# george-gca/sr-pytorch-lightning

Measured on AMD Instinct MI355X. Metric: SR training throughput, LR patches/s (48x48 LR x4, fwd+bwd+Adam), higher is better.
Workload: dtype bf16; 1 GPU; edsr_baseline x4, 48x48 LR patches, batch 256/GPU, train step (L1 + Adam); global_batch=256, parallelism=dp1, hip_graph=full

## Files before the change

### sr-pytorch-lightning_amd/csrc/conv_wgrad.hip

```cpp
#include <stdlib.h>
#include "srk_common.h"

namespace {

template <int DT, int KS> struct WgCfg {
  typedef DTraits<DT> Tr;
  static constexpr int CH = Tr::CH;
  static constexpr int ESZ = 16 / CH;
  static constexpr int CBLK = 128 / ESZ;
  static constexpr int RB = CBLK / 32;
  static constexpr int PAIRS = RB * RB;
  static constexpr int KGROUPS = 4 / PAIRS;
  static constexpr int NT = 256;
  static constexpr int NTAPS = KS * KS;
  static constexpr int PAD = KS / 2;
  static constexpr int TIN = 16 + KS - 1;
  static constexpr int PITCH = (TIN + 1) & ~1;
  static constexpr int XS_BYTES = TIN * PITCH * 128;
  static constexpr int DYS_BYTES = 256 * 128;
  static constexpr int LDS_BYTES = XS_BYTES + DYS_BYTES;
  static constexpr int XPIECES = TIN * TIN * 8;
  static constexpr int DYPIECES = 256 * 8;
};

// ... 52 lines not shown
    int pt = tile;
    const int tX = pt % tilesX;
    pt /= tilesX;
    const int tY = pt % tilesY;
    const int n = pt / tilesY;
    const int y0 = tY * 16, x0 = tX * 16;

    __syncthreads();
#pragma unroll 1
    for (int base = tid; base < C::XPIECES; base += 4 * C::NT) {
      i32x4 v[4];
#pragma unroll
      for (int u = 0; u < 4; ++u) {
        const int i = base + u * C::NT;
        v[u] = i32x4{0, 0, 0, 0};
        if (i < C::XPIECES) {
          const int s = i & 7, p = i >> 3;
          const int iy = p / C::TIN, ix = p - iy * C::TIN;
          const int c = cib * 8 + (s ^ swz(ix));
          const int gy = y0 + iy - C::PAD, gx = x0 + ix - C::PAD;
          if (c < nch_x && gy >= 0 && gy < H && gx >= 0 && gx < W)
            v[u] = gload16(xg + chunk_off(n, gy, gx, H, W, rx, Csx, c * CH, a.x_pitch, a.x_coff));
        }
      }
#pragma unroll
      for (int u = 0; u < 4; ++u) {
        const int i = base + u * C::NT;
        if (i < C::XPIECES) {
          const int s = i & 7, p = i >> 3;
          const int iy = p / C::TIN, ix = p - iy * C::TIN;
          lds_write16(Xs + ((iy * C::PITCH + ix) << 7) + (s << 4), v[u]);
        }
      }
    }
#pragma unroll 1
    for (int base = tid; base < C::DYPIECES; base += 4 * C::NT) {
      i32x4 v[4];
#pragma unroll
      for (int u = 0; u < 4; ++u) {
        const int i = base + u * C::NT;
        const int s = i & 7, p = i >> 3;
        const int iy = p >> 4, ix = p & 15;
        const int c = cob * 8 + (s ^ swz(ix));
        const int gy = y0 + iy, gx = x0 + ix;
        v[u] = i32x4{0, 0, 0, 0};
        if (c < nch_d && gy < H && gx < W)
          v[u] = gload16(dg + chunk_off(n, gy, gx, H, W, rd, Csd, c * CH, a.dy_pitch, a.dy_coff));
      }
#pragma unroll
      for (int u = 0; u < 4; ++u) lds_write16(Ds + ((base + u * C::NT) << 4), v[u]);
    }
    __syncthreads();

    if (a.dbp && cib == 0) {
#pragma unroll 4
      for (int p = b_part; p < 256; p += BPARTS) {
        const char* ad = Ds + (p << 7) + ((((b_c / CH)) ^ swz(p & 15)) << 4) + (b_c % CH) * C::ESZ;
        bsum += Tr::to_f32(*reinterpret_cast<const elem*>(ad));
      }
    }

    if constexpr (Tr::IS16) {
      i32x4 xf[KS][KS];
#pragma unroll
      for (int rr = 0; rr < KS - 1; ++rr)
#pragma unroll
        for (int kw = 0; kw < KS; ++kw)
          xf[rr % KS][kw] = tr_read2(Xs + xoff[kw][0] + rr * (C::PITCH * 128), Xs + xoff[kw][1] + rr * (C::PITCH * 128));
#pragma unroll
      for (int y = 0; y < 16; ++y) {
        const int nr = y + KS - 1;
#pragma unroll
        for (int kw = 0; kw < KS; ++kw)
          xf[nr % KS][kw] = tr_read2(Xs + xoff[kw][0] + nr * (C::PITCH * 128), Xs + xoff[kw][1] + nr * (C::PITCH * 128));
        const i32x4 bf = tr_read2(Ds + doff[0] + y * (16 * 128), Ds + doff[1] + y * (16 * 128));
#pragma unroll
        for (int t = 0; t < C::NTAPS; ++t) {
          const int kh = t / KS, kw = t - kh * KS;
          acc[t] = Tr::mma(xf[(y + kh) % KS][kw], bf, acc[t]);
        }
      }
    } else {
      const int i = lane & 31, hk = lane >> 5;
#pragma unroll 1
      for (int y = kgroup; y < 16; y += C::KGROUPS) {
#pragma unroll 2
        for (int m = 0; m < 8; ++m) {
          const int col = 2 * m + hk;
          const float b = lds_f32(Ds, 16, y, col, i);
#pragma unroll
          for (int t = 0; t < C::NTAPS; ++t) {
            const int kh = t / KS, kw = t - kh * KS;
            const float av = lds_f32(Xs, C::PITCH, y + kh, col + kw, i);
            acc[t] = __builtin_amdgcn_mfma_f32_32x32x2f32(av, b, acc[t], 0, 0, 0);
          }
        }
      }
    }
  }

  const int co = cob * C::CBLK + cbk * 32 + (lane & 31);
  const int hq = lane >> 5;
  if (co < a.Cout) {
#pragma unroll
    for (int t = 0; t < C::NTAPS; ++t) {
#pragma unroll
      for (int e = 0; e < 16; ++e) {
        const int ci = cib * C::CBLK + rb * 32 + (e & 3) + 8 * (e >> 2) + 4 * hq;
        if (ci < a.Cin) atomicAdd(a.dwp + ((size_t)t * a.Cin + ci) * a.Cout + co, acc[t][e]);
      }
    }
  }
  if (a.dbp && cib == 0) {
    const int c = cob * C::CBLK + b_c;
    if (c < a.Cout) atomicAdd(a.dbp + c, bsum);
  }
}


typedef __attribute__((address_space(3))) void lds_void_t;

template <int DT>
SRK_DEV void wgrad_ws_body16(const srk_wgrad_args& a, const int slot, const int cib, const int cob, const int tilesX, const int tilesY,
                           const unsigned x_bytes, const unsigned dy_bytes, const int tq, const int trem, char* const smem) {
  typedef WgCfg<DT, 3> C;
  typedef typename C::Tr Tr;
  typedef typename Tr::elem elem;
  constexpr int CH = C::CH, KS = 3, GT = 256, ESZ = C::ESZ;
  constexpr int NPK = (C::XPIECES + GT - 1) / GT;
  constexpr int NDK = C::DYPIECES / GT;
  constexpr int BUF_BYTES = C::XS_BYTES + C::DYS_BYTES;

  const int tid = threadIdx.x, lane = tid & 63;
  const int wave = __builtin_amdgcn_readfirstlane(tid >> 6);
  const int rb = wave >> 1, cbk = wave & 1;
  const int H = a.H, W = a.W;
  const int nch_x = a.Cin / CH, nch_d = a.Cout / CH;

  const int t0 = slot * tq + min(slot, trem);
  const int nt = tq + (slot < trem ? 1 : 0);

  const i32x4 xrs = make_rsrc4(a.x, x_bytes), drs = make_rsrc4(a.dy, dy_bytes);
  const unsigned lds0 = lds_addr_of(smem);
  int pconst[NPK], pyx[NPK];
#pragma unroll
  for (int k = 0; k < NPK; ++k) {
    const int i = tid + k * GT;
    const int sl = i & 7, p = i >> 3;
    const int iy = p / C::TIN, ix = p - iy * C::TIN;
    const int c = cib * 8 + (sl ^ swz(ix));
    pconst[k] = (((iy - 1) * W + (ix - 1)) * a.x_pitch + a.x_coff + c * CH) * ESZ;
    pyx[k] = (i < C::XPIECES && c < nch_x) ? (((iy - 1) & 0xffff) | ((ix - 1) << 16)) : (int)0x7fff7fff;
  }
  const int rd = a.dy_ps > 1 ? a.dy_ps : 1;
  const int d_ix = (tid >> 3) & 15, d_iy0 = tid >> 7;
  const int d_c = cob * 8 + ((tid & 7) ^ swz(d_ix));
  const bool d_cok = d_c < nch_d;
  int dconst, dkstride;
  {
    const int Csd = a.Cout / (rd * rd);
    const int k0 = d_c * CH;
    const int ij = k0 / Csd, c0 = k0 - ij * Csd;
    const int si = ij / rd, sj = ij - si * rd;
    dconst = (((d_iy0 * rd + si) * (W * rd) + d_ix * rd + sj) * a.dy_pitch + a.dy_coff + c0) * ESZ;
    dkstride = 2 * rd * (W * rd) * a.dy_pitch * ESZ;
  }
  struct TileAddr { int y0, x0, xbase, dbase; bool colok; unsigned Xb; };
  auto tile_addr = [&](int pt, char* Xb) {
    TileAddr t;
    const int tX = pt % tilesX;
    const int q = pt / tilesX;
    const int tY = q % tilesY, n = q / tilesY;
    t.y0 = tY * 16; t.x0 = tX * 16;
    t.xbase = (((n * H + t.y0) * W + t.x0) * a.x_pitch) * ESZ;
    t.dbase = (((n * H * rd + t.y0 * rd) * (W * rd) + t.x0 * rd) * a.dy_pitch) * ESZ;
    t.colok = d_cok && (t.x0 + d_ix < W);
    t.Xb = lds0 + (unsigned)(Xb - smem);
    return t;
  };
  auto dma_x_piece = [&](const TileAddr& t, int k) {
    const int gy = t.y0 + (int)(short)(pyx[k] & 0xffff), gx = t.x0 + (pyx[k] >> 16);
    const bool ok = (unsigned)gy < (unsigned)H && (unsigned)gx < (unsigned)W;
    const unsigned voff = ok ? (unsigned)(t.xbase + pconst[k]) : 0x80000000u;
    if (k < NPK - 1 || tid + k * GT < C::XPIECES)
      dma16_hidden(xrs, voff, __builtin_amdgcn_readfirstlane(t.Xb + ((k * GT + wave * 64) << 4)));
  };
  auto dma_d_piece = [&](const TileAddr& t, int k) {
    const bool ok = t.colok && (t.y0 + d_iy0 + 2 * k < H);
    const unsigned voff = ok ? (unsigned)(t.dbase + dconst + k * dkstride) : 0x80000000u;
    dma16_hidden(drs, voff, __builtin_amdgcn_readfirstlane(t.Xb + C::XS_BYTES + ((k * GT + wave * 64) << 4)));
  };
  auto dma_tile = [&](int pt, char* Xb) {
    const TileAddr t = tile_addr(pt, Xb);
#pragma unroll
    for (int k = 0; k < NPK; ++k) dma_x_piece(t, k);
#pragma unroll
    for (int k = 0; k < NDK; ++k) dma_d_piece(t, k);
  };

  f32x16 acc[9];
#pragma unroll
  for (int t = 0; t < 9; ++t)
#pragma unroll
    for (int e = 0; e < 16; ++e) acc[t][e] = 0.f;
  float bsum8[8] = {0.f, 0.f, 0.f, 0.f, 0.f, 0.f, 0.f, 0.f};
  const bool do_bias = a.dbp != nullptr && cib == 0;
  int xoff[KS][2], doff[2];
#pragma unroll
  for (int kw = 0; kw < KS; ++kw) {
    xoff[kw][0] = tr_lane_off(kw, 0, rb, lane);
    xoff[kw][1] = tr_lane_off(kw, 1, rb, lane);
  }
  doff[0] = tr_lane_off(0, 0, cbk, lane);
  doff[1] = tr_lane_off(0, 1, cbk, lane);

  dma_tile(t0, smem);
#pragma unroll 1
  for (int it = 0; it < nt; ++it) {
    char* const Xs = smem + (it & 1) * BUF_BYTES;
    char* const Ds = Xs + C::XS_BYTES;
    asm volatile("s_waitcnt vmcnt(0)" ::: "memory");
    __builtin_amdgcn_s_barrier();
    const bool more = it + 1 < nt;
    const TileAddr nxt = tile_addr(more ? t0 + it + 1 : t0 + it, smem + ((it + 1) & 1) * BUF_BYTES);

    if (do_bias) {
#pragma unroll
      for (int k = 0; k < 8; ++k) {
        const i32x4 raw = lds_read16(Ds + ((tid + 256 * k) << 4));
        const uint32_t w4[4] = {(uint32_t)raw.x, (uint32_t)raw.y, (uint32_t)raw.z, (uint32_t)raw.w};
#pragma unroll
        for (int i = 0; i < 4; ++i) {
          bsum8[2 * i] += Tr::to_f32((uint16_t)(w4[i] & 0xffff));
          bsum8[2 * i + 1] += Tr::to_f32((uint16_t)(w4[i] >> 16));
        }
      }
    }
    i32x4 xf[4][KS];
#pragma unroll
    for (int rr = 0; rr < 3; ++rr)
#pragma unroll
      for (int kw = 0; kw < KS; ++kw)
        xf[rr][kw] = tr_read2(Xs + xoff[kw][0] + rr * (C::PITCH * 128), Xs + xoff[kw][1] + rr * (C::PITCH * 128));
    i32x4 bf = tr_read2(Ds + doff[0], Ds + doff[1]);
#pragma unroll
    for (int y = 0; y < 16; ++y) {
      i32x4 bfn = bf;
      if (y + 1 < 16) {
        const int nr = y + 3;
#pragma unroll
        for (int kw = 0; kw < KS; ++kw)
          xf[nr & 3][kw] = tr_read2(Xs + xoff[kw][0] + nr * (C::PITCH * 128), Xs + xoff[kw][1] + nr * (C::PITCH * 128));
        bfn = tr_read2(Ds + doff[0] + (y + 1) * (16 * 128), Ds + doff[1] + (y + 1) * (16 * 128));
      }
#pragma unroll
      for (int t = 0; t < 9; ++t) {
        const int kh = t / KS, kw = t - kh * KS;
        acc[t] = Tr::mma(xf[(y + kh) & 3][kw], bf, acc[t]);
        if (t == 1 && 2 * y < NPK && more) dma_x_piece(nxt, 2 * y);
        if (t == 4 && 2 * y + 1 < NPK && more) dma_x_piece(nxt, 2 * y + 1);
        if (t == 7 && y < NDK && more) dma_d_piece(nxt, y);
      }
      bf = bfn;
      __builtin_amdgcn_sched_barrier(0);
    }
  }

  {
    const int co = cob * 64 + cbk * 32 + (lane & 31);
    const int hq = lane >> 5;
    const size_t slab_elems = (size_t)9 * a.Cin * a.Cout;
    const __amdgpu_buffer_rsrc_t srs =
        __builtin_amdgcn_make_buffer_rsrc(a.dwp + (size_t)slot * slab_elems, 0, (unsigned)(slab_elems * 4), 0x00020000);
    const int ci0 = cib * 64 + rb * 32 + 4 * hq;
#pragma unroll
    for (int t = 0; t < 9; ++t) {
#pragma unroll
      for (int e = 0; e < 16; ++e) {
        const int ci = ci0 + (e & 3) + 8 * (e >> 2);
        const unsigned voff = (ci < a.Cin && co < a.Cout) ? (unsigned)(((t * a.Cin + ci) * a.Cout + co) * 4) : 0x80000000u;
        __builtin_amdgcn_raw_buffer_store_b32(__float_as_uint(acc[t][e]), srs, voff, 0, 0);
      }
    }
  }
  if (do_bias) {
    float* const bred = reinterpret_cast<float*>(smem);
    __syncthreads();
#pragma unroll
    for (int e = 0; e < 8; ++e) bred[tid * 8 + e] = bsum8[e];
    __syncthreads();
    if (tid < 64) {
      const int ch = tid >> 3, e = tid & 7;
      float t = 0.f;
      for (int p0 = 0; p0 < 32; ++p0) t += bred[((p0 << 3) + (ch ^ swz(p0 & 15))) * 8 + e];
      const int c = cob * 64 + tid;
      if (c < a.Cout) a.dbp[(size_t)slot * a.Cout + c] = t;
    }
  }
}


constexpr int WS_TH = 8;

template <int DT>
SRK_DEV void wgrad_ws_body8(const srk_wgrad_args& a, const int slot, const int cib, const int cob, const int tilesX, const int tilesY,
                           const unsigned x_bytes, const unsigned dy_bytes, const int tq, const int trem, char* const smem) {
  typedef WgCfg<DT, 3> C;
  typedef typename C::Tr Tr;
  typedef typename Tr::elem elem;
  constexpr int CH = C::CH, KS = 3, GT = 256, ESZ = C::ESZ;
  constexpr int TH = WS_TH, NBUF = 4, AHEAD = NBUF - 1;
  constexpr int XPIECES = (TH + 2) * C::TIN * 8;
  constexpr int NPK = (XPIECES + GT - 1) / GT;
  constexpr int NDK = TH * 16 * 8 / GT;
  constexpr int PPT = NPK + NDK;
  constexpr int XS_PAD = NPK * GT * 16, DYS = TH * 16 * 128;
  constexpr int BUF_BYTES = XS_PAD + DYS;
  static_assert(NBUF * BUF_BYTES <= 160 * 1024, "the ring must fit the LDS");

  const int tid = threadIdx.x, lane = tid & 63;
  const int wave = __builtin_amdgcn_readfirstlane(tid >> 6);
  const int rb = wave >> 1, cbk = wave & 1;
  const int H = a.H, W = a.W;
  const int nch_x = a.Cin / CH, nch_d = a.Cout / CH;

  const int t0 = slot * tq + min(slot, trem);
  const int nt = tq + (slot < trem ? 1 : 0);

  const i32x4 xrs = make_rsrc4(a.x, x_bytes), drs = make_rsrc4(a.dy, dy_bytes);
  const unsigned lds0 = lds_addr_of(smem);
  int pconst[NPK], pyx[NPK];
#pragma unroll
  for (int k = 0; k < NPK; ++k) {
    const int i = tid + k * GT;
    const int sl = i & 7, p = i >> 3;
    const int iy = p / C::TIN, ix = p - iy * C::TIN;
    const int c = cib * 8 + (sl ^ swz(ix));
    pconst[k] = (((iy - 1) * W + (ix - 1)) * a.x_pitch + a.x_coff + c * CH) * ESZ;
    pyx[k] = (i < XPIECES && c < nch_x) ? (((iy - 1) & 0xffff) | ((ix - 1) << 16)) : (int)0x7fff7fff;
  }
  const int rd = a.dy_ps > 1 ? a.dy_ps : 1;
  const int d_ix = (tid >> 3) & 15, d_iy0 = tid >> 7;
  const int d_c = cob * 8 + ((tid & 7) ^ swz(d_ix));
  const bool d_cok = d_c < nch_d;
  int dconst, dkstride;
  {
    const int Csd = a.Cout / (rd * rd);
    const int k0 = d_c * CH;
    const int ij = k0 / Csd, c0 = k0 - ij * Csd;
    const int si = ij / rd, sj = ij - si * rd;
    dconst = (((d_iy0 * rd + si) * (W * rd) + d_ix * rd + sj) * a.dy_pitch + a.dy_coff + c0) * ESZ;
    dkstride = 2 * rd * (W * rd) * a.dy_pitch * ESZ;
  }
  struct TileAddr { int y0, x0, xbase, dbase; bool colok, live; unsigned Xb; };
  auto tile_addr = [&](int it_, char* Xb) {
    TileAddr t;
    t.live = it_ < nt;
    const int pt = t0 + (t.live ? it_ : 0);
    const int tX = pt % tilesX;
    const int q = pt / tilesX;
    const int tY = q % tilesY, n = q / tilesY;
    t.y0 = tY * TH; t.x0 = tX * 16;
    t.xbase = (((n * H + t.y0) * W + t.x0) * a.x_pitch) * ESZ;
    t.dbase = (((n * H * rd + t.y0 * rd) * (W * rd) + t.x0 * rd) * a.dy_pitch) * ESZ;
    t.colok = t.live && d_cok && (t.x0 + d_ix < W);
    t.Xb = lds0 + (unsigned)(Xb - smem);
    return t;
  };
  auto dma_x_piece = [&](const TileAddr& t, int k) {
    const int gy = t.y0 + (int)(short)(pyx[k] & 0xffff), gx = t.x0 + (pyx[k] >> 16);
    const bool ok = t.live && (unsigned)gy < (unsigned)H && (unsigned)gx < (unsigned)W;
    const unsigned voff = ok ? (unsigned)(t.xbase + pconst[k]) : 0x80000000u;
    dma16_hidden(xrs, voff, __builtin_amdgcn_readfirstlane(t.Xb + ((k * GT + wave * 64) << 4)));
  };
  auto dma_d_piece = [&](const TileAddr& t, int k) {
    const bool ok = t.colok && (t.y0 + d_iy0 + 2 * k < H);
    const unsigned voff = ok ? (unsigned)(t.dbase + dconst + k * dkstride) : 0x80000000u;
    dma16_hidden(drs, voff, __builtin_amdgcn_readfirstlane(t.Xb + XS_PAD + ((k * GT + wave * 64) << 4)));
  };
  auto dma_tile = [&](int it_, char* Xb) {
    const TileAddr t = tile_addr(it_, Xb);
#pragma unroll
    for (int k = 0; k < NPK; ++k) dma_x_piece(t, k);
#pragma unroll
    for (int k = 0; k < NDK; ++k) dma_d_piece(t, k);
  };

  f32x16 acc[9];
#pragma unroll
  for (int t = 0; t < 9; ++t)
#pragma unroll
    for (int e = 0; e < 16; ++e) acc[t][e] = 0.f;
  float bsum8[8] = {0.f, 0.f, 0.f, 0.f, 0.f, 0.f, 0.f, 0.f};
  const bool do_bias = a.dbp != nullptr && cib == 0;
  int xoff[KS][2], doff[2];
#pragma unroll
  for (int kw = 0; kw < KS; ++kw) {
    xoff[kw][0] = tr_lane_off(kw, 0, rb, lane);
    xoff[kw][1] = tr_lane_off(kw, 1, rb, lane);
  }
  doff[0] = tr_lane_off(0, 0, cbk, lane);
  doff[1] = tr_lane_off(0, 1, cbk, lane);

#pragma unroll
  for (int k = 0; k < AHEAD; ++k) dma_tile(k, smem + k * BUF_BYTES);
#pragma unroll 1
  for (int it = 0; it < nt; ++it) {
    char* const Xs = smem + (it & (NBUF - 1)) * BUF_BYTES;
    char* const Ds = Xs + XS_PAD;
    asm volatile("s_waitcnt vmcnt(%0)" :: "n"((AHEAD - 1) * PPT) : "memory");
    __builtin_amdgcn_s_barrier();
    constexpr bool more = true;
    const TileAddr nxt = tile_addr(it + AHEAD, smem + ((it + AHEAD) & (NBUF - 1)) * BUF_BYTES);

    if (do_bias) {
#pragma unroll
      for (int k = 0; k < NDK; ++k) {
        const i32x4 raw = lds_read16(Ds + ((tid + 256 * k) << 4));
        const uint32_t w4[4] = {(uint32_t)raw.x, (uint32_t)raw.y, (uint32_t)raw.z, (uint32_t)raw.w};
#pragma unroll
        for (int i = 0; i < 4; ++i) {
          bsum8[2 * i] += Tr::to_f32((uint16_t)(w4[i] & 0xffff));
          bsum8[2 * i + 1] += Tr::to_f32((uint16_t)(w4[i] >> 16));
        }
      }
    }
    i32x4 xf[4][KS];
#pragma unroll
    for (int rr = 0; rr < 3; ++rr)
#pragma unroll
      for (int kw = 0; kw < KS; ++kw)
        xf[rr][kw] = tr_read2(Xs + xoff[kw][0] + rr * (C::PITCH * 128), Xs + xoff[kw][1] + rr * (C::PITCH * 128));
    i32x4 bf = tr_read2(Ds + doff[0], Ds + doff[1]);
#pragma unroll
    for (int y = 0; y < TH; ++y) {
      i32x4 bfn = bf;
      if (y + 1 < TH) {
        const int nr = y + 3;
#pragma unroll
        for (int kw = 0; kw < KS; ++kw)
          xf[nr & 3][kw] = tr_read2(Xs + xoff[kw][0] + nr * (C::PITCH * 128), Xs + xoff[kw][1] + nr * (C::PITCH * 128));
        bfn = tr_read2(Ds + doff[0] + (y + 1) * (16 * 128), Ds + doff[1] + (y + 1) * (16 * 128));
      }
#pragma unroll
      for (int t = 0; t < 9; ++t) {
        const int kh = t / KS, kw = t - kh * KS;
        acc[t] = Tr::mma(xf[(y + kh) & 3][kw], bf, acc[t]);
        if (t == 1 && y < NPK && more) dma_x_piece(nxt, y);
        if (t == 5 && y < NDK && more) dma_d_piece(nxt, y);
      }
      bf = bfn;
      __builtin_amdgcn_sched_barrier(0);
    }
  }

  asm volatile("s_waitcnt vmcnt(0)" ::: "memory");
  {
    const int co = cob * 64 + cbk * 32 + (lane & 31);
    const int hq = lane >> 5;
    const size_t slab_elems = (size_t)9 * a.Cin * a.Cout;
    const __amdgpu_buffer_rsrc_t srs =
        __builtin_amdgcn_make_buffer_rsrc(a.dwp + (size_t)slot * slab_elems, 0, (unsigned)(slab_elems * 4), 0x00020000);
    const int ci0 = cib * 64 + rb * 32 + 4 * hq;
#pragma unroll
    for (int t = 0; t < 9; ++t) {
#pragma unroll
      for (int e = 0; e < 16; ++e) {
        const int ci = ci0 + (e & 3) + 8 * (e >> 2);
        const unsigned voff = (ci < a.Cin && co < a.Cout) ? (unsigned)(((t * a.Cin + ci) * a.Cout + co) * 4) : 0x80000000u;
        __builtin_amdgcn_raw_buffer_store_b32(__float_as_uint(acc[t][e]), srs, voff, 0, 0);
      }
    }
  }
  if (do_bias) {
    float* const bred = reinterpret_cast<float*>(smem);
    __syncthreads();
#pragma unroll
    for (int e = 0; e < 8; ++e) bred[tid * 8 + e] = bsum8[e];
    __syncthreads();
    if (tid < 64) {
      const int ch = tid >> 3, e = tid & 7;
      float t = 0.f;
      for (int p0 = 0; p0 < 32; ++p0) t += bred[((p0 << 3) + (ch ^ swz(p0 & 15))) * 8 + e];
      const int c = cob * 64 + tid;
      if (c < a.Cout) a.dbp[(size_t)slot * a.Cout + c] = t;
    }
  }
}

template <int DT>
__global__ __launch_bounds__(256, 1) void conv_wgrad_ws_kernel(const srk_wgrad_args a, int tilesX, int tilesY, int th,
                                                                unsigned x_bytes, unsigned dy_bytes, int tq, int trem) {
  extern __shared__ __attribute__((aligned(16))) char smem[];
  if (th == WS_TH) wgrad_ws_body8<DT>(a, blockIdx.x, blockIdx.y, blockIdx.z, tilesX, tilesY, x_bytes, dy_bytes, tq, trem, smem);
  else wgrad_ws_body16<DT>(a, blockIdx.x, blockIdx.y, blockIdx.z, tilesX, tilesY, x_bytes, dy_bytes, tq, trem, smem);
}

struct WgJob {
  srk_wgrad_args a;
  int tilesX, tilesY;
  unsigned x_bytes, dy_bytes;
  int tq, trem;
  int ncib, ncob;
  int block0, th;
};

template <int DT>
__global__ __launch_bounds__(256, 1) void conv_wgrad_ws_group_kernel(const WgJob* __restrict__ jobs, const int* __restrict__ block_job) {
  extern __shared__ __attribute__((aligned(16))) char smem[];
#ifndef SRK_WGRAD_XCD_REMAP
#define SRK_WGRAD_XCD_REMAP 1
#endif
  unsigned lb = blockIdx.x;
  if (SRK_WGRAD_XCD_REMAP) {
    const unsigned q = gridDim.x >> 3, r = gridDim.x & 7u, x = blockIdx.x & 7u;
    lb = x * q + (x < r ? x : r) + (blockIdx.x >> 3);
  }
  const int jid = block_job[lb];
  const WgJob j = jobs[jid];
  const int local = (int)lb - j.block0;
  const int per = j.ncib * j.ncob;
  const int slot = local / per, rem = local - slot * per;
  const int cib = rem / j.ncob, cob = rem - cib * j.ncob;
  if (j.th == WS_TH) wgrad_ws_body8<DT>(j.a, slot, cib, cob, j.tilesX, j.tilesY, j.x_bytes, j.dy_bytes, j.tq, j.trem, smem);
  else wgrad_ws_body16<DT>(j.a, slot, cib, cob, j.tilesX, j.tilesY, j.x_bytes, j.dy_bytes, j.tq, j.trem, smem);
}

template <int DT, int CIB, int COB>
__global__ __launch_bounds__(256, 1) void wgrad1x1_ws_kernel(const srk_wgrad_args a, int ntiles, unsigned x_bytes, unsigned dy_bytes,
                                                              int tq, int trem) {
  typedef DTraits<DT> Tr;
  constexpr int CH = Tr::CH, ESZ = 2;
  constexpr int NPL = CIB + COB;
  constexpr int PLANE = 64 * 128;
  constexpr int BUF_BYTES = NPL * PLANE;
  constexpr int NPK = NPL * 2;
  static_assert(Tr::IS16, "16-bit types only");
  extern __shared__ __attribute__((aligned(16))) char smem[];

  const int tid = threadIdx.x, lane = tid & 63;
  const int wave = __builtin_amdgcn_readfirstlane(tid >> 6);
  const int rb = wave >> 1, cbk = wave & 1;
  const int slot = blockIdx.x, cit = blockIdx.y, cot = blockIdx.z;
  const long long P = (long long)a.N * a.H * a.W;
  const int nch_x = a.Cin / CH, nch_d = a.Cout / CH;
  const int t0 = slot * tq + min(slot, trem);
  const int nt = tq + (slot < trem ? 1 : 0);

  const i32x4 xrs = make_rsrc4(a.x, x_bytes), drs = make_rsrc4(a.dy, dy_bytes);
  const unsigned lds0 = lds_addr_of(smem);
  const int px0 = tid >> 3, sl = tid & 7;
  const int cchunk = sl ^ swz(px0 & 15);
  auto dma_tile = [&](int pt, unsigned buf, int k) {
    const int plane = k >> 1;
    const long long p = (long long)pt * 64 + px0 + 32 * (k & 1);
    const bool isx = plane < CIB;
    const int blk = isx ? cit * CIB + plane : cot * COB + (plane - CIB);
    const int chunk = blk * 8 + cchunk;
    const bool ok = p < P && chunk < (isx ? nch_x : nch_d);
    const unsigned voff = ok ? (unsigned)((p * (isx ? a.x_pitch : a.dy_pitch) + (isx ? a.x_coff : a.dy_coff) + chunk * CH) * ESZ) : 0x80000000u;
    dma16_hidden(isx ? xrs : drs, voff, (unsigned)__builtin_amdgcn_readfirstlane((int)(buf + plane * PLANE + (((k & 1) * 256 + wave * 64) << 4))));
  };

  f32x16 acc[CIB][COB];
#pragma unroll
  for (int i = 0; i < CIB; ++i)
#pragma unroll
    for (int o = 0; o < COB; ++o)
#pragma unroll
      for (int e = 0; e < 16; ++e) acc[i][o][e] = 0.f;
  float bsum[COB][8];
#pragma unroll
  for (int o = 0; o < COB; ++o)
#pragma unroll
    for (int e = 0; e < 8; ++e) bsum[o][e] = 0.f;
  const bool do_bias = a.dbp != nullptr && cit == 0;
  int aoff[2], boff[2];
  aoff[0] = tr_lane_off(0, 0, rb, lane);  aoff[1] = tr_lane_off(0, 1, rb, lane);
  boff[0] = tr_lane_off(0, 0, cbk, lane); boff[1] = tr_lane_off(0, 1, cbk, lane);

  if (nt > 0) {
#pragma unroll
    for (int k = 0; k < NPK; ++k) dma_tile(t0, lds0, k);
  }
#pragma unroll 1
  for (int it = 0; it < nt; ++it) {
    const char* const B0 = smem + (it & 1) * BUF_BYTES;
    const unsigned nb = lds0 + ((it + 1) & 1) * BUF_BYTES;
    asm volatile("s_waitcnt vmcnt(0)" ::: "memory");
    __builtin_amdgcn_s_barrier();
    const bool more = it + 1 < nt;
    if (do_bias) {
#pragma unroll
      for (int o = 0; o < COB; ++o)
#pragma unroll
        for (int hf = 0; hf < 2; ++hf) {
          const i32x4 raw = lds_read16(B0 + (CIB + o) * PLANE + ((tid + 256 * hf) << 4));
          const uint32_t w4[4] = {(uint32_t)raw.x, (uint32_t)raw.y, (uint32_t)raw.z, (uint32_t)raw.w};
#pragma unroll
          for (int i = 0; i < 4; ++i) {
            bsum[o][2 * i] += Tr::to_f32((uint16_t)(w4[i] & 0xffff));
            bsum[o][2 * i + 1] += Tr::to_f32((uint16_t)(w4[i] >> 16));
          }
        }
    }
#pragma unroll
    for (int r = 0; r < 4; ++r) {
      i32x4 af[CIB], bf[COB];
#pragma unroll
      for (int i = 0; i < CIB; ++i) af[i] = tr_read2(B0 + i * PLANE + r * 2048 + aoff[0], B0 + i * PLANE + r * 2048 + aoff[1]);
#pragma unroll
      for (int o = 0; o < COB; ++o) bf[o] = tr_read2(B0 + (CIB + o) * PLANE + r * 2048 + boff[0], B0 + (CIB + o) * PLANE + r * 2048 + boff[1]);
      int k = r * (NPK / 4);
#pragma unroll
      for (int i = 0; i < CIB; ++i)
#pragma unroll
        for (int o = 0; o < COB; ++o) {
          acc[i][o] = Tr::mma(af[i], bf[o], acc[i][o]);
          if (more && k < (r + 1) * (NPK / 4) && ((i * COB + o) & 1) == 0) { dma_tile(t0 + it + 1, nb, k); ++k; }
        }
      __builtin_amdgcn_sched_barrier(0);
    }
  }

  {
    const int hq = lane >> 5;
    const size_t slab_elems = (size_t)a.Cin * a.Cout;
    const __amdgpu_buffer_rsrc_t srs =
        __builtin_amdgcn_make_buffer_rsrc(a.dwp + (size_t)slot * slab_elems, 0, (unsigned)(slab_elems * 4), 0x00020000);
#pragma unroll
    for (int i = 0; i < CIB; ++i)
#pragma unroll
      for (int o = 0; o < COB; ++o) {
        const int ci0 = (cit * CIB + i) * 64 + rb * 32 + 4 * hq;
        const int co = (cot * COB + o) * 64 + cbk * 32 + (lane & 31);
#pragma unroll
        for (int e = 0; e < 16; ++e) {
          const int ci = ci0 + (e & 3) + 8 * (e >> 2);
          const unsigned voff = (ci < a.Cin && co < a.Cout) ? (unsigned)((ci * a.Cout + co) * 4) : 0x80000000u;
          __builtin_amdgcn_raw_buffer_store_b32(__float_as_uint(acc[i][o][e]), srs, voff, 0, 0);
        }
      }
  }
  if (do_bias) {
    float* const bred = reinterpret_cast<float*>(smem);
#pragma unroll
    for (int o = 0; o < COB; ++o) {
      __syncthreads();
#pragma unroll
      for (int e = 0; e < 8; ++e) bred[tid * 8 + e] = bsum[o][e];
      __syncthreads();
      if (tid < 64) {
        const int ch = tid >> 3, e = tid & 7;
        float t = 0.f;
        for (int p0 = 0; p0 < 32; ++p0) t += bred[((p0 << 3) + (ch ^ swz(p0 & 15))) * 8 + e];
        const int c = (cot * COB + o) * 64 + tid;
        if (c < a.Cout) a.dbp[(size_t)slot * a.Cout + c] = t;
      }
    }
  }
}

template <int DT, int NBUF>
__global__ __launch_bounds__(256, 1) void wgrad1x1_small_kernel(const srk_wgrad_args a, int ntiles, unsigned x_bytes, unsigned dy_bytes,
                                                                 int tq, int trem) {
  typedef DTraits<DT> Tr;
  constexpr int CH = Tr::CH, ESZ = 2;
  constexpr int PLANE = 64 * 128, BUF_BYTES = 2 * PLANE, NPK = 4;
  static_assert(Tr::IS16, "16-bit types only");
  extern __shared__ __attribute__((aligned(16))) char smem[];
  const int tid = threadIdx.x, lane = tid & 63;
  const int wave = __builtin_amdgcn_readfirstlane(tid >> 6);
  const int rb = wave >> 1, cbk = wave & 1;
  const int slot = blockIdx.x;
  const long long P = (long long)a.N * a.H * a.W;
  const int nch_x = a.Cin / CH, nch_d = a.Cout / CH;
  const int t0 = slot * tq + min(slot, trem);
  const int nt = tq + (slot < trem ? 1 : 0);
  const i32x4 xrs = make_rsrc4(a.x, x_bytes), drs = make_rsrc4(a.dy, dy_bytes);
  const unsigned lds0 = lds_addr_of(smem);
  const int px0 = tid >> 3, sl = tid & 7;
  const int cchunk = sl ^ swz(px0 & 15);
  auto dma_tile = [&](int j) {
    const unsigned buf = lds0 + (unsigned)(j % NBUF) * BUF_BYTES;
#pragma unroll
    for (int k = 0; k < NPK; ++k) {
      const int plane = k >> 1;
      const long long p = (long long)(t0 + j) * 64 + px0 + 32 * (k & 1);
      const bool isx = plane == 0;
      const bool ok = j < nt && p < P && cchunk < (isx ? nch_x : nch_d);
      const unsigned voff = ok ? (unsigned)((p * (isx ? a.x_pitch : a.dy_pitch) + (isx ? a.x_coff : a.dy_coff) + cchunk * CH) * ESZ) : 0x80000000u;
      dma16_hidden(isx ? xrs : drs, voff, (unsigned)__builtin_amdgcn_readfirstlane((int)(buf + plane * PLANE + (((k & 1) * 256 + wave * 64) << 4))));
    }
  };
  f32x16 acc;
#pragma unroll
  for (int e = 0; e < 16; ++e) acc[e] = 0.f;
  float bsum[8] = {0.f, 0.f, 0.f, 0.f, 0.f, 0.f, 0.f, 0.f};
  const bool do_bias = a.dbp != nullptr;
  const int aoff0 = tr_lane_off(0, 0, rb, lane), aoff1 = tr_lane_off(0, 1, rb, lane);
  const int boff0 = tr_lane_off(0, 0, cbk, lane), boff1 = tr_lane_off(0, 1, cbk, lane);
#pragma unroll
  for (int j = 0; j < NBUF - 1; ++j) dma_tile(j);
#pragma unroll 1
  for (int it = 0; it < nt; ++it) {
    const char* const B0 = smem + (it % NBUF) * BUF_BYTES;
    asm volatile("s_waitcnt vmcnt(%0)" :: "n"((NBUF - 2) * NPK) : "memory");
    __builtin_amdgcn_s_barrier();
    dma_tile(it + NBUF - 1);
    if (do_bias) {
#pragma unroll
      for (int hf = 0; hf < 2; ++hf) {
        const i32x4 raw = lds_read16(B0 + PLANE + ((tid + 256 * hf) << 4));
        const uint32_t w4[4] = {(uint32_t)raw.x, (uint32_t)raw.y, (uint32_t)raw.z, (uint32_t)raw.w};
#pragma unroll
        for (int i = 0; i < 4; ++i) {
          bsum[2 * i] += Tr::to_f32((uint16_t)(w4[i] & 0xffff));
          bsum[2 * i + 1] += Tr::to_f32((uint16_t)(w4[i] >> 16));
        }
      }
    }
#pragma unroll
    for (int r = 0; r < 4; ++r) {
      const i32x4 af = tr_read2(B0 + r * 2048 + aoff0, B0 + r * 2048 + aoff1);
      const i32x4 bf = tr_read2(B0 + PLANE + r * 2048 + boff0, B0 + PLANE + r * 2048 + boff1);
      acc = Tr::mma(af, bf, acc);
    }
  }
  asm volatile("s_waitcnt vmcnt(0)" ::: "memory");
  {
    const int hq = lane >> 5;
    const size_t slab_elems = (size_t)a.Cin * a.Cout;
    const __amdgpu_buffer_rsrc_t srs =
        __builtin_amdgcn_make_buffer_rsrc(a.dwp + (size_t)slot * slab_elems, 0, (unsigned)(slab_elems * 4), 0x00020000);
    const int ci0 = rb * 32 + 4 * hq, co = cbk * 32 + (lane & 31);
#pragma unroll
    for (int e = 0; e < 16; ++e) {
      const int ci = ci0 + (e & 3) + 8 * (e >> 2);
      const unsigned voff = (ci < a.Cin && co < a.Cout) ? (unsigned)((ci * a.Cout + co) * 4) : 0x80000000u;
      __builtin_amdgcn_raw_buffer_store_b32(__float_as_uint(acc[e]), srs, voff, 0, 0);
    }
  }
  if (do_bias) {
    float* const bred = reinterpret_cast<float*>(smem);
    __syncthreads();
#pragma unroll
    for (int e = 0; e < 8; ++e) bred[tid * 8 + e] = bsum[e];
    __syncthreads();
    if (tid < 64) {
      const int ch = tid >> 3, e = tid & 7;
      float t = 0.f;
      for (int p0 = 0; p0 < 32; ++p0) t += bred[((p0 << 3) + (ch ^ swz(p0 & 15))) * 8 + e];
      if (tid < a.Cout) a.dbp[(size_t)slot * a.Cout + tid] = t;
    }
  }
}

static void wgrad1x1_shape(const srk_wgrad_args& a, int& cib, int& cob) {
  if (a.Cout >= a.Cin) { cib = 2; cob = 4; } else { cib = 4; cob = 2; }
}
static int wgrad1x1_slabs(const srk_wgrad_args& a) {
  if (a.dtype == SRK_F32 || a.KH != 1 || a.KW != 1 || a.x_ps > 1 || a.dy_ps > 1) return 0;
  static const bool no_ws = srk_dbg_getenv("SRK_NO_WS") != nullptr;
  if (no_ws) return 0;
  const long long P = (long long)a.N * a.H * a.W;
  if (P * a.x_pitch * 2 >= 0x7fff0000LL || P * a.dy_pitch * 2 >= 0x7fff0000LL) return 0;
  int cib, cob;
  wgrad1x1_shape(a, cib, cob);
  const int cit = (a.Cin + 64 * cib - 1) / (64 * cib), cot = (a.Cout + 64 * cob - 1) / (64 * cob);
  static const int cus = [] { int c = srk_device_cus(); return c > 0 ? c : 256; }();
  const long long ntiles = (P + 63) / 64;
  long long slabs = cus / (cit * cot);
  if (slabs < 1) slabs = 1;
  if (slabs > ntiles) slabs = ntiles;
  return (int)slabs;
}

static int ws_tile_height(long long n_images, int H, int W) {
  static const int forced = [] { const char* e = srk_dbg_getenv("SRK_WGRAD_TH"); return e ? atoi(e) : 0; }();
  if (forced == 8 || forced == 16) return forced;
  return n_images * ((H + 15) / 16) * ((W + 15) / 16) >= 1024 ? WS_TH : 16;
}

static int wgrad_ws_slabs(const srk_wgrad_args& a) {
  if (a.KH == 1 && a.KW == 1) return wgrad1x1_slabs(a);
  if (a.KH > 3) return srk_wgrad_lk_ok(a) ? srk_wgrad_lk_slabs(a) : 0;
  if (a.dtype == SRK_F32 || a.KH != 3 || a.KW != 3 || a.x_ps > 1) return 0;
  static const bool no_ws = srk_dbg_getenv("SRK_NO_WS") != nullptr;
  if (no_ws) return 0;
  const int rd = a.dy_ps > 1 ? a.dy_ps : 1;
  const long long xb = (long long)a.N * a.H * a.W * a.x_pitch * 2, db = (long long)a.N * a.H * a.W * rd * rd * a.dy_pitch * 2;
  if (xb >= 0x7fff0000LL || db >= 0x7fff0000LL) return 0;
  const int th = ws_tile_height(a.N, a.H, a.W);
  const long long ntiles = (long long)a.N * ((a.H + th - 1) / th) * ((a.W + 15) / 16);
  const int cib = (a.Cin + 63) / 64, cob = (a.Cout + 63) / 64;
  static const int cus = [] { int c = srk_device_cus(); return c > 0 ? c : 256; }();
  long long slabs = cus / (cib * cob);
  if (slabs < 1) slabs = 1;
  if (slabs > ntiles) slabs = ntiles;
  return (int)slabs;
}

constexpr int WS_LDS_BYTES = 160 * 1024;

template <int DT> int launch_ws(const srk_wgrad_args& a, hipStream_t st, int slabs) {
  typedef WgCfg<DT, 3> C;
  constexpr int LDS = WS_LDS_BYTES;
  static const hipError_t attr = hipFuncSetAttribute(reinterpret_cast<const void*>(&conv_wgrad_ws_kernel<DT>),
                                                     hipFuncAttributeMaxDynamicSharedMemorySize, LDS);
  if (attr != hipSuccess) {
    srk_set_error("srk_conv2d_wgrad(ws): cannot reserve %d bytes of LDS: %s", LDS, hipGetErrorString(attr));
    return (int)attr;
  }
  const int th = ws_tile_height(a.N, a.H, a.W);
  const int tilesX = (a.W + 15) / 16, tilesY = (a.H + th - 1) / th;
  const long long ntiles = (long long)a.N * tilesX * tilesY;
  const int cib = (a.Cin + 63) / 64, cob = (a.Cout + 63) / 64;
  const int rd = a.dy_ps > 1 ? a.dy_ps : 1;
  const unsigned xb = (unsigned)((long long)a.N * a.H * a.W * a.x_pitch * 2);
  const unsigned db = (unsigned)((long long)a.N * a.H * a.W * rd * rd * a.dy_pitch * 2);
  srk_kernel_name = "wgrad_ws";
  hipLaunchKernelGGL((conv_wgrad_ws_kernel<DT>), dim3(slabs, cib, cob), dim3(256), LDS, st, a, tilesX, tilesY, th, xb, db,
                     (int)(ntiles / slabs), (int)(ntiles % slabs));
  SRK_LAUNCH_CHECK();
  return 0;
}

// ... 206 lines not shown
```

Before: 48050 LR patches/s.

## Software-pipeline wgrad tile loop: prefetch next fragments, interleave bias sum, incremental tile addressing

Restructures the 8-row weight-gradient kernel's main loop so the wait and barrier for the next ring buffer sit inside the last MFMA row, and that tile's first LDS fragments are read before the loop iteration ends. The bias reduction becomes a template parameter and is spread across the MFMA sequence instead of running as a separate LDS-read and add phase at the start of each tile. Tile coordinates are now advanced incrementally rather than recomputed with divides and modulos, and the next tile's address is computed mid-loop. The goal is to hide barrier, LDS and scalar-address latency behind matrix work. The cost is higher register pressure and more fragile scheduling.

```diff
diff --git a/sr-pytorch-lightning_amd/csrc/conv_wgrad.hip b/sr-pytorch-lightning_amd/csrc/conv_wgrad.hip
--- a/sr-pytorch-lightning_amd/csrc/conv_wgrad.hip
+++ b/sr-pytorch-lightning_amd/csrc/conv_wgrad.hip
@@ -378,7 +378,9 @@
 
 constexpr int WS_TH = 8;
 
-template <int DT>
+SRK_DEV void add_f32_unpacked(float& s, float v) { asm("v_add_f32_e32 %0, %0, %1" : "+v"(s) : "v"(v)); }
+
+template <int DT, bool BIAS>
 SRK_DEV void wgrad_ws_body8(const srk_wgrad_args& a, const int slot, const int cib, const int cob, const int tilesX, const int tilesY,
                            const unsigned x_bytes, const unsigned dy_bytes, const int tq, const int trem, char* const smem) {
   typedef WgCfg<DT, 3> C;
@@ -429,18 +431,22 @@
     dkstride = 2 * rd * (W * rd) * a.dy_pitch * ESZ;
   }
   struct TileAddr { int y0, x0, xbase, dbase; bool colok, live; unsigned Xb; };
-  auto tile_addr = [&](int it_, char* Xb) {
+  int nx_tX = t0 % tilesX, nx_tY = (t0 / tilesX) % tilesY, nx_n = (t0 / tilesX) / tilesY;
+  auto tile_addr = [&](int it_) {
     TileAddr t;
     t.live = it_ < nt;
-    const int pt = t0 + (t.live ? it_ : 0);
-    const int tX = pt % tilesX;
-    const int q = pt / tilesX;
-    const int tY = q % tilesY, n = q / tilesY;
-    t.y0 = tY * TH; t.x0 = tX * 16;
-    t.xbase = (((n * H + t.y0) * W + t.x0) * a.x_pitch) * ESZ;
-    t.dbase = (((n * H * rd + t.y0 * rd) * (W * rd) + t.x0 * rd) * a.dy_pitch) * ESZ;
+    t.y0 = nx_tY * TH; t.x0 = nx_tX * 16;
+    const int row = nx_n * H + t.y0;
+    t.xbase = ((row * W + t.x0) * a.x_pitch) * ESZ;
+    t.dbase = ((row * rd * (W * rd) + t.x0 * rd) * a.dy_pitch) * ESZ;
     t.colok = t.live && d_cok && (t.x0 + d_ix < W);
-    t.Xb = lds0 + (unsigned)(Xb - smem);
+    t.Xb = lds0 + (unsigned)((it_ & (NBUF - 1)) * BUF_BYTES);
+    const bool wx = nx_tX + 1 == tilesX;
+    nx_tX = wx ? 0 : nx_tX + 1;
+    nx_tY += wx ? 1 : 0;
+    const bool wy = nx_tY == tilesY;
+    nx_tY = wy ? 0 : nx_tY;
+    nx_n += wy ? 1 : 0;
     return t;
   };
   auto dma_x_piece = [&](const TileAddr& t, int k) {
@@ -454,8 +460,8 @@
     const unsigned voff = ok ? (unsigned)(t.dbase + dconst + k * dkstride) : 0x80000000u;
     dma16_hidden(drs, voff, __builtin_amdgcn_readfirstlane(t.Xb + XS_PAD + ((k * GT + wave * 64) << 4)));
   };
-  auto dma_tile = [&](int it_, char* Xb) {
-    const TileAddr t = tile_addr(it_, Xb);
+  auto dma_tile = [&](int it_) {
+    const TileAddr t = tile_addr(it_);
 #pragma unroll
     for (int k = 0; k < NPK; ++k) dma_x_piece(t, k);
 #pragma unroll
@@ -468,7 +474,6 @@
 #pragma unroll
     for (int e = 0; e < 16; ++e) acc[t][e] = 0.f;
   float bsum8[8] = {0.f, 0.f, 0.f, 0.f, 0.f, 0.f, 0.f, 0.f};
-  const bool do_bias = a.dbp != nullptr && cib == 0;
   int xoff[KS][2], doff[2];
 #pragma unroll
   for (int kw = 0; kw < KS; ++kw) {
@@ -477,37 +482,36 @@
   }
   doff[0] = tr_lane_off(0, 0, cbk, lane);
   doff[1] = tr_lane_off(0, 1, cbk, lane);
-
-#pragma unroll
-  for (int k = 0; k < AHEAD; ++k) dma_tile(k, smem + k * BUF_BYTES);
+  i32x4 pxf[3][KS], pbf;
+  auto read_first_frags = [&](const char* Xb) {
+    const char* const Db = Xb + XS_PAD;
+    pbf = tr_read2(Db + doff[0], Db + doff[1]);
+#pragma unroll
+    for (int rr = 0; rr < 3; ++rr)
+#pragma unroll
+      for (int kw = 0; kw < KS; ++kw)
+        pxf[rr][kw] = tr_read2(Xb + xoff[kw][0] + rr * (C::PITCH * 128), Xb + xoff[kw][1] + rr * (C::PITCH * 128));
+  };
+
+#pragma unroll
+  for (int k = 0; k < AHEAD; ++k) dma_tile(k);
+  TileAddr nxt = tile_addr(AHEAD);
+  asm volatile("s_waitcnt vmcnt(%0)" :: "n"((AHEAD - 1) * PPT) : "memory");
+  __builtin_amdgcn_s_barrier();
+  read_first_frags(smem);
 #pragma unroll 1
   for (int it = 0; it < nt; ++it) {
-    char* const Xs = smem + (it & (NBUF - 1)) * BUF_BYTES;
-    char* const Ds = Xs + XS_PAD;
-    asm volatile("s_waitcnt vmcnt(%0)" :: "n"((AHEAD - 1) * PPT) : "memory");
-    __builtin_amdgcn_s_barrier();
-    constexpr bool more = true;
-    const TileAddr nxt = tile_addr(it + AHEAD, smem + ((it + AHEAD) & (NBUF - 1)) * BUF_BYTES);
-
-    if (do_bias) {
-#pragma unroll
-      for (int k = 0; k < NDK; ++k) {
-        const i32x4 raw = lds_read16(Ds + ((tid + 256 * k) << 4));
-        const uint32_t w4[4] = {(uint32_t)raw.x, (uint32_t)raw.y, (uint32_t)raw.z, (uint32_t)raw.w};
-#pragma unroll
-        for (int i = 0; i < 4; ++i) {
-          bsum8[2 * i] += Tr::to_f32((uint16_t)(w4[i] & 0xffff));
-          bsum8[2 * i + 1] += Tr::to_f32((uint16_t)(w4[i] >> 16));
-        }
-      }
-    }
+    const char* const Xs = smem + (it & (NBUF - 1)) * BUF_BYTES;
+    const char* const Ds = Xs + XS_PAD;
+    const char* const Xn = smem + ((it + 1) & (NBUF - 1)) * BUF_BYTES;
     i32x4 xf[4][KS];
 #pragma unroll
     for (int rr = 0; rr < 3; ++rr)
 #pragma unroll
-      for (int kw = 0; kw < KS; ++kw)
-        xf[rr][kw] = tr_read2(Xs + xoff[kw][0] + rr * (C::PITCH * 128), Xs + xoff[kw][1] + rr * (C::PITCH * 128));
-    i32x4 bf = tr_read2(Ds + doff[0], Ds + doff[1]);
+      for (int kw = 0; kw < KS; ++kw) xf[rr][kw] = pxf[rr][kw];
+    i32x4 bf = pbf;
+    i32x4 braw = {0, 0, 0, 0};
+    TileAddr nn = nxt;
 #pragma unroll
     for (int y = 0; y < TH; ++y) {
       i32x4 bfn = bf;
@@ -518,16 +522,36 @@
           xf[nr & 3][kw] = tr_read2(Xs + xoff[kw][0] + nr * (C::PITCH * 128), Xs + xoff[kw][1] + nr * (C::PITCH * 128));
         bfn = tr_read2(Ds + doff[0] + (y + 1) * (16 * 128), Ds + doff[1] + (y + 1) * (16 * 128));
       }
+      const i32x4 bprev = braw;
+      if (BIAS && y < NDK) braw = lds_read16(Ds + ((tid + 256 * y) << 4));
 #pragma unroll
       for (int t = 0; t < 9; ++t) {
         const int kh = t / KS, kw = t - kh * KS;
         acc[t] = Tr::mma(xf[(y + kh) & 3][kw], bf, acc[t]);
-        if (t == 1 && y < NPK && more) dma_x_piece(nxt, y);
-        if (t == 5 && y < NDK && more) dma_d_piece(nxt, y);
+        if (t == 1 && y < NPK) dma_x_piece(nxt, y);
+        if (t == 5 && y < NDK) dma_d_piece(nxt, y);
+        if (BIAS && y >= 1 && y <= NDK && t >= 2 && t != 5 && t <= 6) {
+          const int i = t - 2 - (t > 5 ? 1 : 0);
+          const uint32_t w = (uint32_t)bprev[i];
+          add_f32_unpacked(bsum8[2 * i], Tr::to_f32((uint16_t)(w & 0xffff)));
+          add_f32_unpacked(bsum8[2 * i + 1], Tr::to_f32((uint16_t)(w >> 16)));
+        }
+        if (y == TH - 2 && t == 3) nn = tile_addr(it + 1 + AHEAD);
+        if (y == TH - 1 && t == 0) {
+          __builtin_amdgcn_sched_barrier(0);
+          asm volatile("s_waitcnt lgkmcnt(0)\n\ts_waitcnt vmcnt(%0)" :: "n"((AHEAD - 1) * PPT) : "memory");
+          __builtin_amdgcn_s_barrier();
+          __builtin_amdgcn_sched_barrier(0);
+        }
+        if (y == TH - 1 && t == 1) {
+          __builtin_amdgcn_sched_barrier(0);
+          read_first_frags(Xn);
+        }
       }
       bf = bfn;
       __builtin_amdgcn_sched_barrier(0);
     }
+    nxt = nn;
   }
 
   asm volatile("s_waitcnt vmcnt(0)" ::: "memory");
@@ -548,7 +572,7 @@
       }
     }
   }
-  if (do_bias) {
+  if (BIAS) {
     float* const bred = reinterpret_cast<float*>(smem);
     __syncthreads();
 #pragma unroll
@@ -565,10 +589,17 @@
 }
 
 template <int DT>
+SRK_DEV void wgrad_ws_run8(const srk_wgrad_args& a, const int slot, const int cib, const int cob, const int tilesX, const int tilesY,
+                          const unsigned x_bytes, const unsigned dy_bytes, const int tq, const int trem, char* const smem) {
+  if (a.dbp != nullptr && cib == 0) wgrad_ws_body8<DT, true>(a, slot, cib, cob, tilesX, tilesY, x_bytes, dy_bytes, tq, trem, smem);
+  else wgrad_ws_body8<DT, false>(a, slot, cib, cob, tilesX, tilesY, x_bytes, dy_bytes, tq, trem, smem);
+}
+
+template <int DT>
 __global__ __launch_bounds__(256, 1) void conv_wgrad_ws_kernel(const srk_wgrad_args a, int tilesX, int tilesY, int th,
                                                                 unsigned x_bytes, unsigned dy_bytes, int tq, int trem) {
   extern __shared__ __attribute__((aligned(16))) char smem[];
-  if (th == WS_TH) wgrad_ws_body8<DT>(a, blockIdx.x, blockIdx.y, blockIdx.z, tilesX, tilesY, x_bytes, dy_bytes, tq, trem, smem);
+  if (th == WS_TH) wgrad_ws_run8<DT>(a, blockIdx.x, blockIdx.y, blockIdx.z, tilesX, tilesY, x_bytes, dy_bytes, tq, trem, smem);
   else wgrad_ws_body16<DT>(a, blockIdx.x, blockIdx.y, blockIdx.z, tilesX, tilesY, x_bytes, dy_bytes, tq, trem, smem);
 }
 
@@ -598,7 +629,7 @@
   const int per = j.ncib * j.ncob;
   const int slot = local / per, rem = local - slot * per;
   const int cib = rem / j.ncob, cob = rem - cib * j.ncob;
-  if (j.th == WS_TH) wgrad_ws_body8<DT>(j.a, slot, cib, cob, j.tilesX, j.tilesY, j.x_bytes, j.dy_bytes, j.tq, j.trem, smem);
+  if (j.th == WS_TH) wgrad_ws_run8<DT>(j.a, slot, cib, cob, j.tilesX, j.tilesY, j.x_bytes, j.dy_bytes, j.tq, j.trem, smem);
   else wgrad_ws_body16<DT>(j.a, slot, cib, cob, j.tilesX, j.tilesY, j.x_bytes, j.dy_bytes, j.tq, j.trem, smem);
 }
 
```

New measurement: 48670 LR patches/s, median of 6. 1.3% higher.
